# alpha-davidson/TensorBNN

Measured on AMD Instinct MI355X. Metric: leapfrog steps/sec (whole node), higher is better.
Workload: dtype f32

## Files before the change

### tensorbnn_amd/csrc/kernels_hmc.hpp

```cpp
#pragma once
#include "common.hpp"
#include "update_ops.hpp"

template <int UC = UPD_COLS, int UG = UPD_GROUPS>
__global__ __launch_bounds__(UC * UG) void k_update(
    NetDev nd, int mode, float eps, const float* __restrict__ eta,
    const float* __restrict__ slabs, int nslab, int pitch,
    const float* __restrict__ q_cur, const float* __restrict__ g_cur,
    float* __restrict__ q, float* __restrict__ p, float* __restrict__ g,
    const int* __restrict__ imgmap, float* __restrict__ qimg, float* __restrict__ gd = nullptr, int img_floats = 0,
    const StepCtl* __restrict__ ctl = nullptr, int t = 0)
{
    asm volatile("" :: "s"(mode), "s"(ctl), "s"(slabs), "s"(nslab), "s"(pitch), "s"(eta), "s"(q), "s"(p), "s"(imgmap), "s"(nd.P), "s"(nd.nl));
    if (ctl && mode != UPD_GRAD_ONLY) {
        const StepCtl me = ctl[blockIdx.y];
        eps = me.eps;
        if (t == 0) mode = UPD_FIRST;
        else if (t < me.L) mode = UPD_MID;
        else if (t == me.L) mode = UPD_LAST;
        else return;
    }
    if (blockIdx.y) {
        const size_t c = blockIdx.y, cp = c * (size_t)nd.P;
        eta += c * nd.H; slabs += c * (size_t)nslab * pitch;
// ... 31 lines not shown
        int w = y;
        for (; w + 12 < nslab; w += 16) {
            s0 += src[(size_t)w * pitch]; s1 += src[(size_t)(w + 4) * pitch];
            s2 += src[(size_t)(w + 8) * pitch]; s3 += src[(size_t)(w + 12) * pitch];
        }
        for (; w < nslab; w += 4) s0 += src[(size_t)w * pitch];
    }
    part[y][x] = (s0 + s1) + (s2 + s3);
    __syncthreads();
    if (y == 0 && j < P) {
        const float v = (part[0][x] + part[1][x]) + (part[2][x] + part[3][x]);
        if (out) out[j] = v;
        if (outd) outd[j] = (double)v;
    }
}

__global__ __launch_bounds__(256) void k_shard_pack(int P, const float* __restrict__ row, const double* __restrict__ pstat, int nstat,
                                                     double* __restrict__ buf, double sub) {
    __shared__ double red[4];
    const int j = blockIdx.x * blockDim.x + threadIdx.x;
    if (row && j < P) buf[j] = (double)row[j];
    if (blockIdx.x == 0) {
        double st = 0.0;
        for (int w = threadIdx.x; w < nstat; w += blockDim.x) st += pstat[w];
        st = block_sum(st, red);
        if (threadIdx.x == 0) buf[P] = st - sub;
    }
}
__global__ __launch_bounds__(256) void k_shard_unpack(int P, const double* __restrict__ buf, float* __restrict__ row,
                                                       double* __restrict__ stat_red) {
    const int j = blockIdx.x * blockDim.x + threadIdx.x;
    if (j < P) row[j] = (float)buf[j];
    if (j == 0) stat_red[0] = buf[P];
}

#define LIKC_BLOCKS 64
__global__ __launch_bounds__(256) void k_pois_const(const float* __restrict__ Y, const float* __restrict__ w, long n, int d_out,
                                                     double* __restrict__ out, double r) {
    __shared__ double red[4];
    double c = 0.0, bad = 0.0;
    const long nel = n * d_out;
    const double lgr = r > 0.0 ? lgamma(r) : 0.0;
    for (long el = (long)blockIdx.x * 256 + threadIdx.x; el < nel; el += (long)LIKC_BLOCKS * 256) {
        const float y = Y[el];
        if (!(y >= 0.f && y < INFINITY)) { bad += 1.0; continue; }
        const double wt = w ? (double)w[el / d_out] : 1.0;
        double t = lgamma((double)y + 1.0);
        if (r > 0.0) t += lgr - lgamma((double)y + r);
        c += wt * t;
    }
    c = block_sum(c, red);
    bad = block_sum(bad, red);
    if (threadIdx.x == 0) { out[2 * blockIdx.x] = c; out[2 * blockIdx.x + 1] = bad; }
}

__global__ __launch_bounds__(256) void k_copy_f32(int n, const float* __restrict__ src, float* __restrict__ dst) {
    const int j = blockIdx.x * blockDim.x + threadIdx.x;
    if (j < n) dst[j] = src[j];
}

__global__ __launch_bounds__(256) void k_make_image(int P, const float* __restrict__ q,
                                                    const int* __restrict__ imgmap, float* __restrict__ qimg,
                                                    long q_stride = 0, long img_stride = 0) {
    q += (size_t)blockIdx.y * q_stride; qimg += (size_t)blockIdx.y * img_stride;
    const int j = blockIdx.x * blockDim.x + threadIdx.x;
    if (j < P) { const float v = q[j]; qimg[imgmap[j]] = v; const int m1 = imgmap[P + j]; if (m1 >= 0) qimg[m1] = v; }
}

__device__ __forceinline__ double data_logp(const NetDev& nd, const float* __restrict__ eta, double stat, double n, double lik_c) {
    if (nd.lik == TBNN_LIK_POISSON) return stat - lik_c;
    if (nd.lik == TBNN_LIK_NEG_BINOMIAL) return stat - lik_c;
    if (nd.lik == TBNN_LIK_BERNOULLI || nd.lik == TBNN_LIK_CATEGORICAL) return stat;
    if (nd.lik == TBNN_LIK_HETERO_GAUSSIAN) return stat - 0.5 * 1.8378770664093453  * n;
    if (nd.lik == TBNN_LIK_STUDENT_T) {
        const double nu = (double)nd.lik_df, s = (double)lik_sigma(nd, eta);
        const double c = lgamma(0.5 * (nu + 1.0)) - lgamma(0.5 * nu) - 0.5 * log(nu * 3.14159265358979323846) - log(s);
        return n * (double)nd.d_out * c - 0.5 * (nu + 1.0) * stat;
    }
    const double s = (double)lik_sigma(nd, eta);
    const double nel = (double)n * (double)nd.d_out;
    return -0.5 * (2.0 * nel * log(s) + stat / (s * s) + nel * 1.8378770664093453 );
}

__device__ __forceinline__ double prior_logp_partial(const NetDev& nd, const float* __restrict__ eta,
                                                     const float* __restrict__ q) {
    double acc = 0.0;
    for (int l = 0; l < nd.nl; ++l) {
        for (int part = 0; part < 2; ++part) {
            const int off = part ? nd.offB[l] : nd.offW[l];
            const int cnt = part ? nd.out[l] : nd.out[l] * nd.in[l];
            const float loc = eta[4 * l + 2 * part];
            const float gg = eta[4 * l + 2 * part + 1];
            const float scale = gg * gg;
            if (nd.prior[l] == TBNN_PRIOR_CAUCHY) {
                const float lb = logf(3.14159265358979323846f * scale);
                for (int e = threadIdx.x; e < cnt; e += blockDim.x) {
                    const float z = (q[off + e] - loc) / scale;
                    acc += (double)(logf(1.f + z * z) - lb);
                }
            } else {
                const float s = fminf(fmaxf(scale, 1e-8f), 1e8f);
                for (int e = threadIdx.x; e < cnt; e += blockDim.x) {
                    const float d = (q[off + e] - loc) / s;
                    acc += -0.5 * (double)(d * d);
                }
                if (threadIdx.x == 0) acc += -0.5 * (2.0 * (double)logf(s) + 1.8378770664093453);
            }
        }
    }
    return acc;
}

__global__ __launch_bounds__(1024) void k_begin(
    NetDev nd, const float* __restrict__ p0_inj, const float* __restrict__ logu_inj,
    uint32_t epoch, uint32_t key0, uint32_t key1, float* __restrict__ p, Scal* __restrict__ sc, uint32_t seed_hi = 0)
{
    __shared__ double red[16];
    if (blockIdx.y) {
        const uint32_t c = blockIdx.y;
        key1 = (((key1 ^ seed_hi) + c) ^ seed_hi);
        p += (size_t)c * nd.P; sc += c;
        if (p0_inj) p0_inj += (size_t)c * nd.P;
        if (logu_inj) logu_inj += c;
    }
    double k = 0.0;
    if (p0_inj) {
        for (int j = threadIdx.x; j < nd.P; j += blockDim.x) { const float v = p0_inj[j]; p[j] = v; k += (double)v * (double)v; }
    } else {
        for (int b = threadIdx.x; 4 * b < nd.P; b += blockDim.x) {
            float v[4];
            philox_normal4((uint32_t)b, epoch, PURPOSE_MOMENTUM, key0, key1, v);
#pragma unroll
            for (int i = 0; i < 4; ++i)
                if (4 * b + i < nd.P) { p[4 * b + i] = v[i]; k += (double)v[i] * (double)v[i]; }
        }
    }
    k = block_sum(k, red);
    if (threadIdx.x == 0) {
        sc->k0 = 0.5 * k;
        sc->logu = logu_inj ? (double)logu_inj[0] : (double)philox_logu(epoch, PURPOSE_LOGU, key0, key1);
    }
}

enum { EN_CUR = 0, EN_NEW = 1, EN_TRACE = 2, EN_REFRESH = 3 };
__global__ __launch_bounds__(1024) void k_energy(
    NetDev nd, int which, const float* __restrict__ eta, const float* __restrict__ q,
    const float* __restrict__ p, const float* q_cur,
    const double* __restrict__ partial_stat, int nslab, double n, double lik_c,
    Scal* __restrict__ sc, double* __restrict__ trace_slot,
    Scal* __restrict__ commit_out = nullptr, const float* __restrict__ g = nullptr, float* q_cur_w = nullptr,
    float* __restrict__ g_cur = nullptr, const float* __restrict__ gd = nullptr, float* __restrict__ gd_cur = nullptr,
    const Scal* __restrict__ only_if_accepted = nullptr)
{
    __shared__ double red[16];
    __shared__ int s_acc;
    if (only_if_accepted && !only_if_accepted[blockIdx.y].accepted) return;
    if (blockIdx.y) {
        const size_t c = blockIdx.y, cp = c * (size_t)nd.P;
        eta += c * nd.H; q += cp; p += cp; q_cur += cp; partial_stat += c * PSTAT_CAP; sc += c;
        if (commit_out) commit_out += c;
        if (g) g += cp;
        if (q_cur_w) q_cur_w += cp;
        if (g_cur) g_cur += cp;
        if (gd) gd += cp;
        if (gd_cur) gd_cur += cp;
    }
    double st = 0.0;
    if (which != EN_REFRESH) {
        for (int w = threadIdx.x; w < nslab; w += blockDim.x) st += partial_stat[w];
        st = block_sum(st, red);
    }
    double pr = prior_logp_partial(nd, eta, q);
    pr = block_sum(pr, red);
    double k1 = 0.0, d2 = 0.0;
    if (which == EN_NEW) {
        for (int j = threadIdx.x; j < nd.P; j += blockDim.x) {
            const double pj = (double)p[j];
            const double dq = (double)q[j] - (double)q_cur[j];
            k1 += pj * pj;
            d2 += dq * dq;
        }
        k1 = block_sum(k1, red);
        d2 = block_sum(d2, red);
    }
    const bool commit = which == EN_NEW && commit_out != nullptr;
    if (threadIdx.x != 0 && !commit) return;
    if (threadIdx.x == 0) {
        if (which == EN_REFRESH) { st = sc->stat_cur; which = EN_CUR; }
        const double lp = pr + data_logp(nd, eta, st, n, lik_c);
        if (which == EN_TRACE) { *trace_slot = lp; return; }
        if (which == EN_CUR) {
            sc->stat_cur = st; sc->prior_cur = pr; sc->logp_cur = lp;
            if (trace_slot) *trace_slot = lp;
            return;
        }
        sc->stat_new = st; sc->prior_new = pr; sc->logp_new = lp;
        sc->k1 = 0.5 * k1; sc->d2 = d2;
        double lar = lp - sc->logp_cur + sc->k0 - 0.5 * k1;
        if (!isfinite(lar)) lar = -INFINITY;
        sc->lar = lar;
        const int acc = sc->logu < lar ? 1 : 0;
        sc->accepted = acc;
        sc->sjd = acc ? d2 : 0.0;
        if (trace_slot) *trace_slot = lp;
        if (commit) {
            *commit_out = *sc;
            if (acc) { sc->stat_cur = st; sc->prior_cur = pr; sc->logp_cur = lp; }
            s_acc = acc;
        }
    }
    if (!commit) return;
    __syncthreads();
    if (!s_acc) return;
    for (int j = threadIdx.x; j < nd.P; j += blockDim.x) { q_cur_w[j] = q[j]; g_cur[j] = g[j]; gd_cur[j] = gd[j]; }
}

__global__ __launch_bounds__(256) void k_commit(
    int P, const Scal* __restrict__ sc, const float* __restrict__ q, const float* __restrict__ g,
    float* __restrict__ q_cur, float* __restrict__ g_cur, const float* __restrict__ gd, float* __restrict__ gd_cur)
{
    const size_t c = blockIdx.y, cp = c * (size_t)P;
    if (!sc[c].accepted) return;
    const int j = blockIdx.x * blockDim.x + threadIdx.x;
    if (j < P) { q_cur[cp + j] = q[cp + j]; g_cur[cp + j] = g[cp + j]; gd_cur[cp + j] = gd[cp + j]; }
}

__global__ __launch_bounds__(256) void k_refresh_grad_after_hyper(
    NetDev nd, const float* __restrict__ eta, const float* __restrict__ q_cur,
    const float* __restrict__ gd_cur, float* __restrict__ g_cur, const Scal* __restrict__ hyper_rec = nullptr)
{
    if (blockIdx.y) {
        const size_t c = blockIdx.y, cp = c * (size_t)nd.P;
        eta += c * nd.H; q_cur += cp; gd_cur += cp; g_cur += cp;
    }
    if (hyper_rec && !hyper_rec[blockIdx.y].accepted) return;
    const int j = blockIdx.x * blockDim.x + threadIdx.x;
    if (j >= nd.P) return;
    const float sn = lik_sigma(nd, eta);
    const float inv_var = nd.lik == TBNN_LIK_GAUSSIAN ? 1.f / (sn * sn) : 1.f;
    int prior; float loc, scale;
    prior_params(nd, eta, j, prior, loc, scale);
    g_cur[j] = gd_cur[j] * inv_var + prior_grad(prior, loc, scale, q_cur[j]);
}
__global__ void k_commit_scal(Scal* __restrict__ sc, Scal* __restrict__ host_copy) {
    if (threadIdx.x != 0) return;
    sc += blockIdx.x; host_copy += blockIdx.x;
    *host_copy = *sc;
    if (sc->accepted) { sc->stat_cur = sc->stat_new; sc->prior_cur = sc->prior_new; sc->logp_cur = sc->logp_new; }
}

__global__ void k_trace_logp_cur(const Scal* __restrict__ sc, double* __restrict__ slot) {
    if (threadIdx.x == 0 && blockIdx.x == 0) *slot = sc->logp_cur;
}

__global__ void k_debug_draw(uint32_t epoch, uint32_t purpose, uint32_t key0, uint32_t key1, int n,
                             float* __restrict__ normals, float* __restrict__ logu) {
    const int j = blockIdx.x * blockDim.x + threadIdx.x;
    if (j < n) normals[j] = philox_normal((uint32_t)j, epoch, purpose, key0, key1);
    if (j == 0) logu[0] = philox_logu(epoch, purpose + 1u, key0, key1);
}
```

### tensorbnn_amd/csrc/tbnn_api.hip

```cpp
#include <hip/hip_runtime.h>
#include <rccl/rccl.h>
#include <dlfcn.h>
#include <cmath>
#include <cstdio>
#include <cstdlib>
#include <cstring>
#include <memory>
#include <new>
#include <string>
#include <utility>
#include <vector>

#include "common.hpp"
#include "kernels_generic.hpp"
#include "kernels_hmc.hpp"
#include "kernels_hyper.hpp"
#include "kernels_layered.hpp"
#include "kernels_ensemble.hpp"
#include "kernels_optim.hpp"
#include "aot_ops.hpp"
#include <mutex>

static thread_local std::string g_err;
static int fail(int code, const std::string& msg) { g_err = msg; return code; }
// ... 611 lines not shown
    HIPCHK(hipMemcpyAsync(h->tmp + h->nd.P, h->eta, (size_t)h->nd.H * sizeof(float), hipMemcpyDeviceToDevice, h->stream));
    NCCLCHK(g_rccl.AllGather(h->tmp, d_out, per, ncclFloat, c->comm, h->stream));
    if (host_out) HIPCHK(hipMemcpyAsync(host_out, d_out, tot * sizeof(float), hipMemcpyDeviceToHost, h->stream));
    HIPCHK(hipStreamSynchronize(h->stream));
    return 0;
}
extern "C" int tbnn_set_row_shard(tbnn_handle h, tbnn_comm_handle c, int64_t n_total) {
    NEED(h);
    ONE_CHAIN(h, "tbnn_set_row_shard");
    HIPCHK(hipSetDevice(h->device));
    HIPCHK(hipStreamSynchronize(h->stream));
    if (c && n_total < 1) return fail(-1, "n_total must be >= 1");
    if (c && h->dYw) return fail(-1, "tbnn_set_row_shard: the handle has row weights (tbnn_set_row_weights): weighted row sharding needs the weight sum of all ranks");
    h->shard = c; h->n_total = c ? (long)n_total : 0;
    h->cur_valid = false;
    return 0;
}
static inline double rows_total(const tbnn_ctx* h) { return h->dYw ? h->wsum : (double)(h->shard ? h->n_total : h->n); }
static inline double lik_const(const tbnn_ctx* h) { return h->shard ? 0.0 : h->lik_c; }
static inline const float* pass_Y(const tbnn_ctx* h) { return h->dYw ? h->dYw : h->dY; }
static inline const float* pass_w(const tbnn_ctx* h) { return h->dYw ? h->dYw + (size_t)h->n * h->nd.d_out : nullptr; }
static inline int stat_entries(const tbnn_ctx* h) { return h->shard ? 1 : h->grid; }
static inline const double* stat_ptr(const tbnn_ctx* h) { return h->shard ? h->pstat_red : h->pstat; }
static inline const float* grad_slabs(const tbnn_ctx* h) { return (h->shard && !h->be->slab_is_grad_row()) ? h->grow : h->slabs; }
static inline int grad_nslab(const tbnn_ctx* h) { return h->shard ? 1 : h->nslab; }

static hipEvent_t profile_begin(tbnn_ctx* h, int steps) {
    if (!(h->profile > 0 && (h->launch_no++ % h->profile) == 0)) return nullptr;
    if (h->pev_used + 2 > h->pev.size()) {
        hipEvent_t a = nullptr, b = nullptr;
        hipEventCreate(&a); hipEventCreate(&b); h->pev.emplace_back(a); h->pev.emplace_back(b);
    }
    const hipEvent_t a = h->pev[h->pev_used], b = h->pev[h->pev_used + 1];
    h->pev_used += 2;
    h->pev_div.push_back(steps);
    hipEventRecord(a, h->stream);
    return b;
}
static int launch_fwd_bwd(tbnn_ctx* h, const float* q, const float* eta, const StepCtl* ctl = nullptr, int t = 0) {
    const float* img = nullptr;
    const int C = h->C;
    const long imgS = h->img_floats, slabS = (long)h->nslab * h->pitch;
    if (h->imgmap) {
        if (q == h->q && h->q_img_valid) img = h->qimg;
        else {
            hipLaunchKernelGGL(k_make_image, dim3((h->nd.P + 255) / 256, C), dim3(256), 0, h->stream, h->nd.P, q, h->imgmap, h->qimg_cur, (long)h->nd.P, imgS);
            img = h->qimg_cur;
        }
    }
    const hipEvent_t prof_end = profile_begin(h, 1);
    const PassArgs pa = {img, imgS, q, eta, (long)h->nd.H, h->dX, pass_Y(h), pass_w(h), h->n, h->slabs, slabS, h->pitch, h->pstat, C, ctl, t, h->ctl_host};
    if (const int rc = h->be->fwd_bwd(h->stream, pa)) return rc;
    if (h->shard) {
        const bool dense = h->be->slab_is_grad_row();
        float* row = dense ? h->slabs : h->grow;
        const int P = h->nd.P;
        if (!dense)
            hipLaunchKernelGGL(k_slab_reduce, dim3((P + 63) / 64), dim3(64, 4), 0, h->stream, (const float*)h->slabs, h->nslab,
                               h->pitch, P, (float*)nullptr, h->shard_buf);
        hipLaunchKernelGGL(k_shard_pack, dim3((P + 255) / 256), dim3(256), 0, h->stream, P, dense ? (const float*)row : (const float*)nullptr,
                           (const double*)h->pstat, h->grid, h->shard_buf, h->lik_c);
        NCCLCHK(g_rccl.AllReduce(h->shard_buf, h->shard_buf, (size_t)P + 1, ncclDouble, ncclSum, h->shard->comm, h->stream));
        hipLaunchKernelGGL(k_shard_unpack, dim3((P + 255) / 256), dim3(256), 0, h->stream, P, (const double*)h->shard_buf, row, h->pstat_red);
    }
    if (prof_end) hipEventRecord(prof_end, h->stream);
    HIPCHK(hipGetLastError());
    return 0;
}
static void launch_update(tbnn_ctx* h, int mode, float eps, const float* eta, float* q, float* g, const StepCtl* ctl = nullptr, int t = 0) {
    const bool big = h->nd.P >= UPD_BIG_P;
    const int ucols = big ? UPD_COLS_BIG : UPD_COLS;
    const int gx = (h->pitch / 4 + ucols - 1) / ucols;
    const bool img = h->imgmap && q == h->q;
    float* gd = g == h->g_cur ? h->gd_cur : (g == h->g ? h->gd : nullptr);
    if (big)
        hipLaunchKernelGGL((k_update<UPD_COLS_BIG, UPD_GROUPS_BIG>), dim3(gx, h->C), dim3(UPD_COLS_BIG, UPD_GROUPS_BIG), 0, h->stream, h->nd, mode, eps, eta,
                           grad_slabs(h), grad_nslab(h), h->pitch, h->q_cur, h->g_cur, q, h->p, g, img ? h->imgmap : nullptr, h->qimg, gd, h->img_floats, ctl, t);
    else
        hipLaunchKernelGGL((k_update<UPD_COLS, UPD_GROUPS>), dim3(gx, h->C), dim3(UPD_COLS, UPD_GROUPS), 0, h->stream, h->nd, mode, eps, eta, grad_slabs(h),
                           grad_nslab(h), h->pitch, h->q_cur, h->g_cur, q, h->p, g, img ? h->imgmap : nullptr, h->qimg, gd, h->img_floats, ctl, t);
    if (img && (mode == UPD_FIRST || mode == UPD_MID)) h->q_img_valid = true;
}
static void launch_energy(tbnn_ctx* h, int which, const float* eta, const float* q, double* slot) {
    hipLaunchKernelGGL(k_energy, dim3(1, h->C), dim3(1024), 0, h->stream, h->nd, which, eta, q, h->p, h->q_cur, stat_ptr(h),
                       stat_entries(h), rows_total(h), lik_const(h), h->sc, slot);
}

static int ensure_current(tbnn_ctx* h, double* slot) {
    if (h->cur_valid) return 0;
    int rc = launch_fwd_bwd(h, h->q_cur, h->eta);
    if (rc) return rc;
    launch_update(h, UPD_GRAD_ONLY, 0.f, h->eta, h->q_cur, h->g_cur);
    launch_energy(h, EN_CUR, h->eta, h->q_cur, slot);
    h->cur_valid = true;
    return 0;
}
static float drain_profile(tbnn_ctx* h) {
    double tot = 0.0; int cnt = 0;
    for (size_t i = 0; i + 1 < h->pev_used; i += 2) {
        float ms = 0.f;
        const int div = i / 2 < h->pev_div.size() ? h->pev_div[i / 2] : 1;
        if (hipEventElapsedTime(&ms, h->pev[i], h->pev[i + 1]) == hipSuccess) { tot += ms * 1000.0 / (div > 0 ? div : 1); ++cnt; }
    }
    h->pev_used = 0;
    h->pev_div.clear();
    return cnt ? (float)(tot / cnt) : 0.f;
}

static int stage_theta(tbnn_ctx* h, const float* theta, const float** dq) {
    *dq = h->q_cur;
    if (!theta) return 0;
    HIPCHK(hipMemcpyAsync(h->q, theta, (size_t)h->nd.P * sizeof(float), hipMemcpyHostToDevice, h->stream));
    *dq = h->q; h->q_img_valid = false;
    return 0;
}

extern "C" int tbnn_logp_grad(tbnn_handle h, const float* theta, const float* eta, double* logp, float* grad,
                              double* stat) {
    NEED(h);
    ONE_CHAIN(h, "tbnn_logp_grad");
    if (!h->dX) return fail(-1, "tbnn_set_data has not been called");
    HIPCHK(hipSetDevice(h->device));
    const NetDev& nd = h->nd;
    const float* dq = nullptr;
    const float* de = h->eta;
    if (const int rc = stage_theta(h, theta, &dq)) return rc;
    if (eta) { HIPCHK(hipMemcpyAsync(h->tmp + nd.P, eta, (size_t)nd.H * sizeof(float), hipMemcpyHostToDevice, h->stream)); de = h->tmp + nd.P; }
    int rc = launch_fwd_bwd(h, dq, de);
    if (rc) return rc;
    const int gx = (h->pitch / 4 + UPD_COLS - 1) / UPD_COLS;
    hipLaunchKernelGGL((k_update<UPD_COLS, UPD_GROUPS>), dim3(gx), dim3(UPD_COLS, UPD_GROUPS), 0, h->stream, nd, (int)UPD_GRAD_ONLY, 0.f, de, grad_slabs(h), grad_nslab(h),
                       h->pitch, h->q_cur, h->g_cur, const_cast<float*>(dq), h->p, h->tmp, (const int*)nullptr, (float*)nullptr, (float*)nullptr);
    HIPCHK(h->trace.grow(2, 4096));
    hipLaunchKernelGGL(k_energy, dim3(1), dim3(1024), 0, h->stream, nd, (int)EN_TRACE, de, dq, h->p, h->q_cur, stat_ptr(h),
                       stat_entries(h), rows_total(h), lik_const(h), h->sc, h->trace);
    HIPCHK(hipGetLastError());
    double lp = 0.0;
    HIPCHK(hipMemcpyAsync(&lp, h->trace, sizeof(double), hipMemcpyDeviceToHost, h->stream));
    if (grad) HIPCHK(hipMemcpyAsync(grad, h->tmp, (size_t)nd.P * sizeof(float), hipMemcpyDeviceToHost, h->stream));
    std::vector<double> ps;
    if (stat) { ps.resize(stat_entries(h)); HIPCHK(hipMemcpyAsync(ps.data(), stat_ptr(h), ps.size() * sizeof(double), hipMemcpyDeviceToHost, h->stream)); }
    HIPCHK(hipStreamSynchronize(h->stream));
    if (h->profile) drain_profile(h);
    if (logp) *logp = lp;
    if (stat) {
        double s = 0; for (double v : ps) s += v;
        *stat = s - lik_const(h);
        if (nd.lik == TBNN_LIK_HETERO_GAUSSIAN) *stat -= 0.5 * 1.8378770664093453  * rows_total(h);
    }
    return 0;
}

extern "C" int tbnn_forward(tbnn_handle h, const float* theta, const float* X, int64_t n, float* out) {
    NEED(h);
    if (!theta) ONE_CHAIN(h, "tbnn_forward at the chain's own state");
    if (!X || !out || n < 1) return fail(-1, "forward: null pointer or n < 1");
    HIPCHK(hipSetDevice(h->device));
    const NetDev& nd = h->nd;
    const float* dq = nullptr;
    if (const int rc = stage_theta(h, theta, &dq)) return rc;
    Buf<float> dXf, dOut;
    HIPCHK(dXf.alloc((size_t)n * nd.d_in));
    HIPCHK(dOut.alloc((size_t)n * nd.d_out));
    HIPCHK(hipMemcpyAsync(dXf, X, (size_t)n * nd.d_in * sizeof(float), hipMemcpyHostToDevice, h->stream));
    if (const int rc = h->be->forward(h->stream, 1, dq, dXf, (long)n, dOut, h->imgmap, h->qimg_cur)) return rc;
    HIPCHK(hipMemcpyAsync(out, dOut, (size_t)n * nd.d_out * sizeof(float), hipMemcpyDeviceToHost, h->stream));
    HIPCHK(hipStreamSynchronize(h->stream));
    return 0;
}

extern "C" int tbnn_set_validation(tbnn_handle h, const float* X, const float* Y, int64_t n) {
    NEED(h);
    if (!X || !Y || n < 1) return fail(-1, "set_validation: null pointer or n < 1");
    HIPCHK(hipSetDevice(h->device));
    HIPCHK(hipStreamSynchronize(h->stream));
    h->dXv.reset(); h->dYv.reset();
    HIPCHK(h->dXv.alloc((size_t)n * h->nd.d_in));
    HIPCHK(h->dYv.alloc((size_t)n * h->nd.d_out));
    HIPCHK(hipMemcpy(h->dXv, X, (size_t)n * h->nd.d_in * sizeof(float), hipMemcpyHostToDevice));
    HIPCHK(hipMemcpy(h->dYv, Y, (size_t)n * h->nd.d_out * sizeof(float), hipMemcpyHostToDevice));
    h->nv = (long)n;
    return 0;
}

static int predict_resident(tbnn_ctx* h, int which, const float* theta, long* n_out) {
    const NetDev& nd = h->nd;
    if (!theta) ONE_CHAIN(h, "tbnn_predict / tbnn_metrics at the chain's own state");
    const float* dX = which ? h->dXv : h->dX;
    const long n = which ? h->nv : h->n;
    if (!dX || n < 1) return fail(-1, which ? "tbnn_set_validation has not been called" : "tbnn_set_data has not been called");
    const float* dq = nullptr;
    if (const int rc = stage_theta(h, theta, &dq)) return rc;
    const size_t need = (size_t)n * nd.d_out;
    HIPCHK(h->fbuf.grow(need, need));
    *n_out = n;
    return h->be->forward(h->stream, 1, dq, dX, n, h->fbuf, h->imgmap, h->qimg_cur);
}

extern "C" int tbnn_predict(tbnn_handle h, int which, const float* theta, float* out) {
    NEED(h);
    if (which != 0 && which != 1) return fail(-1, "which must be 0 (training rows) or 1 (validation rows)");
    HIPCHK(hipSetDevice(h->device));
    long n = 0;
    int rc = predict_resident(h, which, theta, &n);
    if (rc) return rc;
    if (out) HIPCHK(hipMemcpyAsync(out, h->fbuf, (size_t)n * h->nd.d_out * sizeof(float), hipMemcpyDeviceToHost, h->stream));
    HIPCHK(hipStreamSynchronize(h->stream));
    return 0;
}

#include "ensemble_api.hpp"

extern "C" int tbnn_metrics(tbnn_handle h, int which, const float* theta, float mean, float sd, int exp_pred, int exp_real,
                            double out3[3]) {
    NEED(h);
    if (!out3) return fail(-1, "null out3");
    if (which != 0 && which != 1) return fail(-1, "which must be 0 (training rows) or 1 (validation rows)");
    HIPCHK(hipSetDevice(h->device));
    long n = 0;
    int rc = predict_resident(h, which, theta, &n);
    if (rc) return rc;
    const int MB = 256;
    HIPCHK(h->mpart.grow(3 * MB, 3 * MB));
    const int d_cmp = h->nd.lik == TBNN_LIK_HETERO_GAUSSIAN ? 1 : h->nd.d_out;
    const long tot = n * d_cmp;
    const int grid = (int)std::min<long>(MB, (tot + 255) / 256);
    hipLaunchKernelGGL(k_metrics, dim3(grid), dim3(256), 0, h->stream, (const float*)h->fbuf, (const float*)(which ? h->dYv : h->dY), n,
                       d_cmp, h->nd.d_out, mean, sd, exp_pred, exp_real, h->mpart);
    HIPCHK(hipGetLastError());
    std::vector<double> part(3 * (size_t)grid);
    HIPCHK(hipMemcpyAsync(part.data(), h->mpart, part.size() * sizeof(double), hipMemcpyDeviceToHost, h->stream));
    HIPCHK(hipStreamSynchronize(h->stream));
    double a[3] = {0, 0, 0};
    for (int b = 0; b < grid; ++b) for (int k = 0; k < 3; ++k) a[k] += part[3 * b + k];
    for (int k = 0; k < 3; ++k) out3[k] = a[k] / (double)tot;
    return 0;
}

static int enqueue_transition(tbnn_ctx* h, float eps, int L, const float* d_p0, const float* d_logu, double* d_trace,
                              Scal* d_out, const StepCtl* ctl = nullptr) {
    const NetDev& nd = h->nd;
    const bool cached = h->cur_valid;
    int rc = ensure_current(h, d_trace);
    if (rc) return rc;
    if (d_trace && cached) hipLaunchKernelGGL(k_trace_logp_cur, dim3(1), dim3(64), 0, h->stream, (const Scal*)h->sc, d_trace);
    hipLaunchKernelGGL(k_begin, dim3(1, h->C), dim3(1024), 0, h->stream, nd, d_p0, d_logu, h->epoch, h->key0, h->key1, h->p, h->sc, h->seed_hi);
    launch_update(h, UPD_FIRST, eps, h->eta, h->q, h->g, ctl, 0);
    const bool traj = h->traj && !d_trace && L >= 1 && h->n <= h->be->traj_max_rows() && !h->shard;
    h->last_path = traj ? "trajectory" : "per-step";
    if (traj) {
        const hipEvent_t prof_end = profile_begin(h, L);
        const int trc = h->be->trajectory(h->stream, h->C, h->qimg, (long)h->img_floats, h->eta, h->dX, h->dY, h->n, h->q, h->p, h->g, h->gd, h->imgmap, h->pstat,
                                          stat_entries(h), eps, L, ctl);
        if (prof_end) hipEventRecord(prof_end, h->stream);
        if (trc)
            return fail(-2, "trajectory kernel launch failed");
        h->q_img_valid = false;
    }
    for (int t = 1; t <= L && !traj; ++t) {
        rc = launch_fwd_bwd(h, h->q, h->eta, ctl, t);
        if (rc) return rc;
        if (d_trace && t < L) {
            launch_update(h, UPD_GRAD_ONLY, 0.f, h->eta, h->q, h->g);
            launch_energy(h, EN_TRACE, h->eta, h->q, d_trace + t);
        }
        launch_update(h, t < L ? UPD_MID : UPD_LAST, eps, h->eta, h->q, h->g, ctl, t);
    }
    if (h->merge_ends && nd.P <= 32768) {
        hipLaunchKernelGGL(k_energy, dim3(1, h->C), dim3(1024), 0, h->stream, h->nd, (int)EN_NEW, (const float*)h->eta, (const float*)h->q, (const float*)h->p,
                           (const float*)h->q_cur, stat_ptr(h), stat_entries(h), rows_total(h), lik_const(h), h->sc, d_trace ? d_trace + L : (double*)nullptr,
                           d_out, (const float*)h->g, h->q_cur, h->g_cur, (const float*)h->gd, h->gd_cur);
    } else {
        launch_energy(h, EN_NEW, h->eta, h->q, d_trace ? d_trace + L : nullptr);
        hipLaunchKernelGGL(k_commit, dim3((nd.P + 255) / 256, h->C), dim3(256), 0, h->stream, nd.P, (const Scal*)h->sc, (const float*)h->q, (const float*)h->g,
                           h->q_cur, h->g_cur, (const float*)h->gd, h->gd_cur);
        hipLaunchKernelGGL(k_commit_scal, dim3(h->C), dim3(64), 0, h->stream, h->sc, d_out);
    }
    HIPCHK(hipGetLastError());
    h->epoch += 1;
    return 0;
}

static void fill_out(const Scal& s, int L, float dev_us, float fb_us, tbnn_step_out* o) {
    o->accepted = s.accepted; o->n_leapfrog = L;
    o->log_accept_ratio = (float)s.lar;
    o->accept_prob = s.lar < 0 ? (float)exp(s.lar) : 1.f;
    o->logp_old = s.logp_cur; o->logp_new = s.logp_new;
    o->kinetic_old = s.k0; o->kinetic_new = s.k1;
    o->sjd = s.sjd; o->device_us = dev_us; o->fwdbwd_us = fb_us;
}

extern "C" int tbnn_hmc_step(tbnn_handle h, float eps, int32_t L, const float* p0, const float* log_u,
                             tbnn_step_out* out, double* trace_logp) {
    NEED(h);
    if (!h->dX) return fail(-1, "tbnn_set_data has not been called");
    if (L < 1) return fail(-1, "L must be >= 1");
    if (h->C > 1 && (p0 || log_u || trace_logp)) return fail(-1, "hmc_step on a multi-chain handle: no injected draws, no trace (out: one record per chain)");
    HIPCHK(hipSetDevice(h->device));
    const NetDev& nd = h->nd;
    const float* d_p0 = nullptr; const float* d_lu = nullptr;
    if (p0) { HIPCHK(hipMemcpyAsync(h->p0_inj, p0, (size_t)nd.P * sizeof(float), hipMemcpyHostToDevice, h->stream)); d_p0 = h->p0_inj; }
    if (log_u) { HIPCHK(hipMemcpyAsync(h->logu_inj, log_u, sizeof(float), hipMemcpyHostToDevice, h->stream)); d_lu = h->logu_inj; }
    double* d_trace = nullptr;
    if (trace_logp) {
        HIPCHK(h->trace.grow((size_t)L + 1, (size_t)L + 1 + 4096));
        d_trace = h->trace;
    }
    HIPCHK(hipEventRecord(h->ev0, h->stream));
    int rc = enqueue_transition(h, eps, L, d_p0, d_lu, d_trace, h->sc_out);
    if (rc) return rc;
    HIPCHK(hipEventRecord(h->ev1, h->stream));
    HIPCHK(hipMemcpyAsync(h->sc_host, h->sc_out, (size_t)h->C * sizeof(Scal), hipMemcpyDeviceToHost, h->stream));
    if (trace_logp) HIPCHK(hipMemcpyAsync(trace_logp, h->trace, (size_t)(L + 1) * sizeof(double), hipMemcpyDeviceToHost, h->stream));
    HIPCHK(hipStreamSynchronize(h->stream));
    float ms = 0.f; hipEventElapsedTime(&ms, h->ev0, h->ev1);
    const float fb = h->profile ? drain_profile(h) : 0.f;
    if (out)
        for (int c = 0; c < h->C; ++c) fill_out(h->sc_host[c], L, ms * 1000.f, fb, out + c);
    return 0;
}

static int grow_records(tbnn_ctx* h, int n_epochs) {
    const size_t need = (size_t)n_epochs * h->C;
    HIPCHK(h->d_recs.grow(need, std::max<size_t>(need, 64)));
    HIPCHK(h->h_recs.grow(need, std::max<size_t>(need, 64)));
    return 0;
}
extern "C" int tbnn_hmc_run(tbnn_handle h, float eps, int32_t L, int32_t n_epochs, tbnn_step_out* outs) {
    NEED(h);
    if (!h->dX) return fail(-1, "tbnn_set_data has not been called");
    if (L < 1 || n_epochs < 1) return fail(-1, "L and n_epochs must be >= 1");
    if ((long long)n_epochs * (long long)h->C > (1LL << 24)) return fail(-1, "n_epochs x chains exceeds 2^24 records per call: split the run");
    HIPCHK(hipSetDevice(h->device));
    const int C = h->C;
    if (const int rc = grow_records(h, n_epochs)) return rc;
    HIPCHK(hipEventRecord(h->ev0, h->stream));
    for (int e = 0; e < n_epochs; ++e) {
        int rc = enqueue_transition(h, eps, L, nullptr, nullptr, nullptr, h->d_recs + (size_t)e * C);
        if (rc) return rc;
    }
    HIPCHK(hipEventRecord(h->ev1, h->stream));
    HIPCHK(hipMemcpyAsync(h->h_recs, h->d_recs, (size_t)n_epochs * C * sizeof(Scal), hipMemcpyDeviceToHost, h->stream));
    HIPCHK(hipStreamSynchronize(h->stream));
    float ms = 0.f; hipEventElapsedTime(&ms, h->ev0, h->ev1);
    const float fb = h->profile ? drain_profile(h) : 0.f;
    if (outs)
        for (int c = 0; c < C; ++c)
            for (int e = 0; e < n_epochs; ++e) fill_out(h->h_recs[(size_t)e * C + c], L, ms * 1000.f / n_epochs, fb, outs + (size_t)c * n_epochs + e);
    return 0;
}

static int stage_ctl(tbnn_ctx* h, const float* eps, const int32_t* L, int* Lmax) {
// ... 150 lines not shown
    const size_t B = (size_t)h->C * h->nd.P * sizeof(float);
    if (m) HIPCHK(hipMemcpyAsync(m, h->opt_m, B, hipMemcpyDeviceToHost, h->stream));
    if (v) HIPCHK(hipMemcpyAsync(v, h->opt_v, B, hipMemcpyDeviceToHost, h->stream));
    if (vhat) HIPCHK(hipMemcpyAsync(vhat, h->opt_vhat, B, hipMemcpyDeviceToHost, h->stream));
    if (g) HIPCHK(hipMemcpyAsync(g, h->opt_g, B, hipMemcpyDeviceToHost, h->stream));
    HIPCHK(hipStreamSynchronize(h->stream));
    if (t) *t = (int32_t)h->opt_t;
    return 0;
}

extern "C" int tbnn_hyper_logp_grad(tbnn_handle h, const float* eta, double* logp, float* grad) {
    NEED(h);
    ONE_CHAIN(h, "tbnn_hyper_logp_grad");
    if (!h->dX) return fail(-1, "tbnn_set_data has not been called");
    HIPCHK(hipSetDevice(h->device));
    const NetDev& nd = h->nd;
    int rc = ensure_current(h, nullptr);
    if (rc) return rc;
    float* de = h->eta;
    if (eta) { HIPCHK(hipMemcpyAsync(h->tmp + nd.P, eta, (size_t)nd.H * sizeof(float), hipMemcpyHostToDevice, h->stream)); de = h->tmp + nd.P; }
    hipLaunchKernelGGL(k_hyper, dim3(1), dim3(HYP_THREADS), 0, h->stream, nd, (int)HYP_EVAL, 0.f, 0, de, h->q_cur, rows_total(h),
                       (const float*)nullptr, (const float*)nullptr, 0u, h->key0, h->key1, h->sc, h->hyp_ws, h->sc_out);
    HIPCHK(hipGetLastError());
    std::vector<float> ws(hyper_ws_bytes(nd) / sizeof(float));
    HIPCHK(hipMemcpyAsync(ws.data(), h->hyp_ws, hyper_ws_bytes(nd), hipMemcpyDeviceToHost, h->stream));
    HIPCHK(hipMemcpyAsync(h->sc_host, h->sc_out, sizeof(Scal), hipMemcpyDeviceToHost, h->stream));
    HIPCHK(hipStreamSynchronize(h->stream));
    if (logp) *logp = h->sc_host[0].logp_new;
    if (grad) memcpy(grad, ws.data() + HYP_WS_GRAD * nd.H, (size_t)nd.H * sizeof(float));
    return 0;
}

static int hyper_step_impl(tbnn_handle h, float eps_h, const float* eps_each, int32_t L_h, const float* p0, const float* log_u, tbnn_step_out* out);
extern "C" int tbnn_hyper_step(tbnn_handle h, float eps_h, int32_t L_h, const float* p0, const float* log_u,
                               tbnn_step_out* out) {
    return hyper_step_impl(h, eps_h, nullptr, L_h, p0, log_u, out);
}
extern "C" int tbnn_hyper_step_each(tbnn_handle h, const float* eps_h, int32_t L_h, tbnn_step_out* out) {
    NEED(h);
    if (!eps_h) return fail(-1, "null eps_h array");
    return hyper_step_impl(h, 0.f, eps_h, L_h, nullptr, nullptr, out);
}
static int hyper_step_impl(tbnn_handle h, float eps_h, const float* eps_each, int32_t L_h, const float* p0, const float* log_u, tbnn_step_out* out) {
    NEED(h);
    if (!h->dX) return fail(-1, "tbnn_set_data has not been called");
    if (L_h < 1) return fail(-1, "L_h must be >= 1");
    if (h->C > 1 && (p0 || log_u)) return fail(-1, "hyper_step on a multi-chain handle: no injected draws (out: one record per chain)");
    HIPCHK(hipSetDevice(h->device));
    const NetDev& nd = h->nd;
    const int C = h->C;
    int rc = ensure_current(h, nullptr);
    if (rc) return rc;
    const float* d_p0 = nullptr; const float* d_lu = nullptr;
    if (p0) { HIPCHK(hipMemcpyAsync(h->p0_inj, p0, (size_t)nd.H * sizeof(float), hipMemcpyHostToDevice, h->stream)); d_p0 = h->p0_inj; }
    if (log_u) { HIPCHK(hipMemcpyAsync(h->logu_inj, log_u, sizeof(float), hipMemcpyHostToDevice, h->stream)); d_lu = h->logu_inj; }
    HIPCHK(hipMemcpyAsync(h->eta_prev, h->eta, (size_t)C * nd.H * sizeof(float), hipMemcpyDeviceToDevice, h->stream));
    const float* d_each = nullptr;
    if (eps_each) {
        memcpy(h->epsh_host, eps_each, (size_t)C * sizeof(float));
        HIPCHK(hipMemcpyAsync(h->epsh, h->epsh_host, (size_t)C * sizeof(float), hipMemcpyHostToDevice, h->stream));
        d_each = h->epsh;
    }
    HIPCHK(hipEventRecord(h->ev0, h->stream));
    const uint32_t ep = h->epoch > 0 ? h->epoch - 1 : 0;
    static_assert(sizeof(float) * 4 == 16, "hyper work space: 4 H floats per chain (hyper_ws_bytes)");
    hipLaunchKernelGGL(k_hyper, dim3(C), dim3(HYP_THREADS), 0, h->stream, nd, (int)HYP_STEP, eps_h, (int)L_h, h->eta, (const float*)h->q_cur, rows_total(h),
                       d_p0, d_lu, ep, h->key0, h->key1, h->sc, h->hyp_ws, h->sc_out, h->seed_hi, d_each);
    HIPCHK(hipGetLastError());
    HIPCHK(hipEventRecord(h->ev1, h->stream));
    HIPCHK(hipMemcpyAsync(h->sc_host, h->sc_out, (size_t)C * sizeof(Scal), hipMemcpyDeviceToHost, h->stream));
    HIPCHK(hipStreamSynchronize(h->stream));
    float ms = 0.f; hipEventElapsedTime(&ms, h->ev0, h->ev1);
    if (out)
        for (int c = 0; c < C; ++c) fill_out(h->sc_host[c], L_h, ms * 1000.f, 0.f, out + c);
    bool any = false;
    for (int c = 0; c < C; ++c) any = any || h->sc_host[c].accepted;
    if (any) {
        static const bool full = getenv("TBNN_HYPER_FULL_REFRESH") && atoi(getenv("TBNN_HYPER_FULL_REFRESH"));
        if (full || !h->cur_valid) h->cur_valid = false;
        else {
            const Scal* gate = C > 1 ? (const Scal*)h->sc_out : (const Scal*)nullptr;
            hipLaunchKernelGGL(k_refresh_grad_after_hyper, dim3((nd.P + 255) / 256, C), dim3(256), 0, h->stream, nd,
                               (const float*)h->eta, (const float*)h->q_cur, (const float*)h->gd_cur, h->g_cur, gate);
            hipLaunchKernelGGL(k_energy, dim3(1, C), dim3(1024), 0, h->stream, nd, (int)EN_REFRESH, (const float*)h->eta,
                               (const float*)h->q_cur, (const float*)h->p, (const float*)h->q_cur,
                               stat_ptr(h), stat_entries(h), rows_total(h), lik_const(h), h->sc, (double*)nullptr,
                               (Scal*)nullptr, (const float*)nullptr, (float*)nullptr, (float*)nullptr, (const float*)nullptr, (float*)nullptr, gate);
            HIPCHK(hipGetLastError());
        }
    }
    return 0;
}

extern "C" int tbnn_hyper_probs_many(tbnn_handle h, const int32_t* priors, const float* thetas, int64_t theta_stride,
                                     const float* etas, int64_t eta_stride, int32_t m, double* out) {
    NEED(h);
    const NetDev& nd0 = h->nd;
    if (!thetas || !etas || !out || m < 1 || theta_stride < nd0.P || eta_stride < 4 * nd0.nl)
        return fail(-1, "hyper_probs_many: null pointer, m < 1, theta_stride < P or eta_stride < 4 * layers");
    NetDev nd = nd0;
    if (priors)
        for (int l = 0; l < nd.nl; ++l) {
            if (priors[l] != TBNN_PRIOR_CAUCHY && priors[l] != TBNN_PRIOR_GAUSSIAN) return fail(-1, "hyper_probs_many: unknown prior");
            nd.prior[l] = priors[l];
        }
    HIPCHK(hipSetDevice(h->device));
    Buf<float> dTh, dEt; Buf<double> dOut;
    const int chunk = (int)std::min<size_t>((size_t)m, std::max<size_t>(1, ((size_t)1 << 28) / (size_t)nd.P));
    HIPCHK(dTh.alloc((size_t)chunk * nd.P));
    HIPCHK(dEt.alloc((size_t)chunk * 4 * nd.nl));
    HIPCHK(dOut.alloc((size_t)chunk));
    for (int i0 = 0; i0 < m; i0 += chunk) {
        const int c = std::min(chunk, m - i0);
        HIPCHK(hipMemcpy2DAsync(dTh, (size_t)nd.P * sizeof(float), thetas + (size_t)i0 * theta_stride, (size_t)theta_stride * sizeof(float),
                                (size_t)nd.P * sizeof(float), (size_t)c, hipMemcpyHostToDevice, h->stream));
        HIPCHK(hipMemcpy2DAsync(dEt, (size_t)4 * nd.nl * sizeof(float), etas + (size_t)i0 * eta_stride, (size_t)eta_stride * sizeof(float),
                                (size_t)4 * nd.nl * sizeof(float), (size_t)c, hipMemcpyHostToDevice, h->stream));
        hipLaunchKernelGGL(k_hyper_probs, dim3(c), dim3(256), 0, h->stream, nd, (const float*)dTh, (long)nd.P, (const float*)dEt, (long)(4 * nd.nl), dOut);
        HIPCHK(hipGetLastError());
        HIPCHK(hipMemcpyAsync(out + i0, dOut, (size_t)c * sizeof(double), hipMemcpyDeviceToHost, h->stream));
        HIPCHK(hipStreamSynchronize(h->stream));
    }
    return 0;
}

extern "C" int tbnn_export_sample_device(tbnn_handle h, float* d_out) {
    NEED(h); if (!d_out) return fail(-1, "null d_out");
    ONE_CHAIN(h, "tbnn_export_sample_device");
    HIPCHK(hipSetDevice(h->device));
    HIPCHK(hipMemcpyAsync(d_out, h->q_cur, (size_t)h->nd.P * sizeof(float), hipMemcpyDeviceToDevice, h->stream));
    HIPCHK(hipMemcpyAsync(d_out + h->nd.P, h->eta, (size_t)h->nd.H * sizeof(float), hipMemcpyDeviceToDevice, h->stream));
    HIPCHK(hipStreamSynchronize(h->stream));
    return 0;
}

extern "C" int tbnn_debug_momentum(tbnn_handle h, float* p_out) {
    NEED(h); if (!p_out) return fail(-1, "null p_out");
    ONE_CHAIN(h, "tbnn_debug_momentum");
    HIPCHK(hipSetDevice(h->device));
    HIPCHK(hipMemcpyAsync(p_out, h->p, (size_t)h->nd.P * sizeof(float), hipMemcpyDeviceToHost, h->stream));
    HIPCHK(hipStreamSynchronize(h->stream));
    return 0;
}

extern "C" int tbnn_debug_draw(tbnn_handle h, uint32_t epoch, uint32_t purpose, int32_t n, float* out_normals,
                               float* out_log_u) {
    NEED(h);
    if (n < 1 || !out_normals) return fail(-1, "debug_draw: bad arguments");
    HIPCHK(hipSetDevice(h->device));
    Buf<float> d;
    HIPCHK(d.alloc((size_t)n + 1));
    hipLaunchKernelGGL(k_debug_draw, dim3((n + 255) / 256), dim3(256), 0, h->stream, epoch, purpose, h->key0, h->key1, (int)n, d, d + n);
    HIPCHK(hipGetLastError());
    std::vector<float> host(n + 1);
    HIPCHK(hipMemcpyAsync(host.data(), d, (size_t)(n + 1) * sizeof(float), hipMemcpyDeviceToHost, h->stream));
    HIPCHK(hipStreamSynchronize(h->stream));
    memcpy(out_normals, host.data(), (size_t)n * sizeof(float));
    if (out_log_u) *out_log_u = host[n];
    return 0;
}

extern "C" int tbnn_debug_stamps(tbnn_handle h, uint64_t* out5) {
    if (!out5) return fail(-1, "null out16");
    NEED(h);
    const FusedOps* ops = h->be->ops();
    if (!ops || ops != narrow_find(h->nd) || !h->dX || h->C > 1) return fail(-1, "debug_stamps: narrow fast kernel + data required");
    HIPCHK(hipSetDevice(h->device));
// ... 55 lines not shown
```

Baseline: 22220.

## Preload energy-kernel operands into registers and shared memory, fuse block reductions

Restructures k_energy so each thread issues all of its global loads (q, p, q_cur, g, gd, eta, partial stats, Scal) up front into register arrays, stages q and eta in shared memory for the prior pass, and merges the separate block reductions into one multi-value reduction. The commit copy reuses the register-held values instead of reloading them. k_begin gets the same early-load treatment. The goal is to cut the serialized global-load latency and the repeated __syncthreads reductions in a single-block-per-chain kernel, at the cost of more registers and about 24KB of shared memory per block.

```diff
diff --git a/tensorbnn_amd/csrc/kernels_hmc.hpp b/tensorbnn_amd/csrc/kernels_hmc.hpp
--- a/tensorbnn_amd/csrc/kernels_hmc.hpp
+++ b/tensorbnn_amd/csrc/kernels_hmc.hpp
@@ -137,8 +137,8 @@
     return -0.5 * (2.0 * nel * log(s) + stat / (s * s) + nel * 1.8378770664093453 );
 }
 
-__device__ __forceinline__ double prior_logp_partial(const NetDev& nd, const float* __restrict__ eta,
-                                                     const float* __restrict__ q) {
+template <class QAt>
+__device__ __forceinline__ double prior_logp_partial_of(const NetDev& nd, const float* __restrict__ eta, QAt qat, int stride) {
     double acc = 0.0;
     for (int l = 0; l < nd.nl; ++l) {
         for (int part = 0; part < 2; ++part) {
@@ -149,14 +149,14 @@
             const float scale = gg * gg;
             if (nd.prior[l] == TBNN_PRIOR_CAUCHY) {
                 const float lb = logf(3.14159265358979323846f * scale);
-                for (int e = threadIdx.x; e < cnt; e += blockDim.x) {
-                    const float z = (q[off + e] - loc) / scale;
+                for (int e = threadIdx.x; e < cnt; e += stride) {
+                    const float z = (qat(off + e) - loc) / scale;
                     acc += (double)(logf(1.f + z * z) - lb);
                 }
             } else {
                 const float s = fminf(fmaxf(scale, 1e-8f), 1e8f);
-                for (int e = threadIdx.x; e < cnt; e += blockDim.x) {
-                    const float d = (q[off + e] - loc) / s;
+                for (int e = threadIdx.x; e < cnt; e += stride) {
+                    const float d = (qat(off + e) - loc) / s;
                     acc += -0.5 * (double)(d * d);
                 }
                 if (threadIdx.x == 0) acc += -0.5 * (2.0 * (double)logf(s) + 1.8378770664093453);
@@ -165,12 +165,41 @@
     }
     return acc;
 }
+__device__ __forceinline__ double prior_logp_partial(const NetDev& nd, const float* __restrict__ eta,
+                                                     const float* __restrict__ q) {
+    return prior_logp_partial_of(nd, eta, [q](int i) { return q[i]; }, (int)blockDim.x);
+}
+
+#define EN_THREADS 1024
+#define EN_CAP 6
+static_assert(EN_CAP == 6, "EN_PIN names the elements");
+#define EN_PIN(a) asm volatile("" : "+v"(a[0]), "+v"(a[1]), "+v"(a[2]), "+v"(a[3]), "+v"(a[4]), "+v"(a[5]))
+
+template <int N, int NW = EN_THREADS / 64>
+__device__ __forceinline__ void block_sum_n(double (&v)[N], double (*red)[16]) {
+    const int lane = threadIdx.x & 63, w = threadIdx.x >> 6, nw = NW;
+#pragma unroll
+    for (int i = 0; i < N; ++i) v[i] = wave_sum(v[i]);
+    if (lane == 0) {
+#pragma unroll
+        for (int i = 0; i < N; ++i) red[i][w] = v[i];
+    }
+    __syncthreads();
+#pragma unroll
+    for (int i = 0; i < N; ++i) v[i] = 0.0;
+    if (w == 0) {
+#pragma unroll
+        for (int i = 0; i < N; ++i) v[i] = lane < nw ? red[i][lane] : 0.0;
+#pragma unroll
+        for (int i = 0; i < N; ++i) v[i] = wave_sum(v[i]);
+    }
+}
 
 __global__ __launch_bounds__(1024) void k_begin(
     NetDev nd, const float* __restrict__ p0_inj, const float* __restrict__ logu_inj,
     uint32_t epoch, uint32_t key0, uint32_t key1, float* __restrict__ p, Scal* __restrict__ sc, uint32_t seed_hi = 0)
 {
-    __shared__ double red[16];
+    __shared__ double red[1][16];
     if (blockIdx.y) {
         const uint32_t c = blockIdx.y;
         key1 = (((key1 ^ seed_hi) + c) ^ seed_hi);
@@ -178,11 +207,19 @@
         if (p0_inj) p0_inj += (size_t)c * nd.P;
         if (logu_inj) logu_inj += c;
     }
+    double logu = 0.0;
+    if (threadIdx.x == 0) logu = logu_inj ? (double)logu_inj[0] : (double)philox_logu(epoch, PURPOSE_LOGU, key0, key1);
     double k = 0.0;
     if (p0_inj) {
-        for (int j = threadIdx.x; j < nd.P; j += blockDim.x) { const float v = p0_inj[j]; p[j] = v; k += (double)v * (double)v; }
+        float v[EN_CAP];
+#pragma unroll
+        for (int i = 0; i < EN_CAP; ++i) { const int j = threadIdx.x + i * EN_THREADS; v[i] = j < nd.P ? p0_inj[j] : 0.f; }
+        EN_PIN(v);
+#pragma unroll
+        for (int i = 0; i < EN_CAP; ++i) { const int j = threadIdx.x + i * EN_THREADS; if (j < nd.P) { p[j] = v[i]; k += (double)v[i] * (double)v[i]; } }
+        for (int j = threadIdx.x + EN_CAP * EN_THREADS; j < nd.P; j += EN_THREADS) { const float x = p0_inj[j]; p[j] = x; k += (double)x * (double)x; }
     } else {
-        for (int b = threadIdx.x; 4 * b < nd.P; b += blockDim.x) {
+        for (int b = threadIdx.x; 4 * b < nd.P; b += EN_THREADS) {
             float v[4];
             philox_normal4((uint32_t)b, epoch, PURPOSE_MOMENTUM, key0, key1, v);
 #pragma unroll
@@ -190,10 +227,11 @@
                 if (4 * b + i < nd.P) { p[4 * b + i] = v[i]; k += (double)v[i] * (double)v[i]; }
         }
     }
-    k = block_sum(k, red);
+    double kv[1] = {k};
+    block_sum_n<1>(kv, red);
     if (threadIdx.x == 0) {
-        sc->k0 = 0.5 * k;
-        sc->logu = logu_inj ? (double)logu_inj[0] : (double)philox_logu(epoch, PURPOSE_LOGU, key0, key1);
+        sc->k0 = 0.5 * kv[0];
+        sc->logu = logu;
     }
 }
 
@@ -207,8 +245,12 @@
     float* __restrict__ g_cur = nullptr, const float* __restrict__ gd = nullptr, float* __restrict__ gd_cur = nullptr,
     const Scal* __restrict__ only_if_accepted = nullptr)
 {
-    __shared__ double red[16];
+    __shared__ double red[4][16];
     __shared__ int s_acc;
+    __shared__ float s_q[EN_CAP * EN_THREADS];
+    __shared__ float s_eta[4 * TBNN_MAX_LAYERS + 4];
+    asm volatile("" :: "s"(which), "s"(eta), "s"(q), "s"(p), "s"(q_cur), "s"(partial_stat), "s"(nslab), "s"(sc), "s"(commit_out), "s"(g), "s"(gd),
+                 "s"(only_if_accepted), "s"(nd.P), "s"(nd.H), "s"(nd.nl), "s"(nd.offW[0]), "s"(nd.offB[0]), "s"(nd.out[0]), "s"(nd.in[0]), "s"(nd.prior[0]));
     if (only_if_accepted && !only_if_accepted[blockIdx.y].accepted) return;
     if (blockIdx.y) {
         const size_t c = blockIdx.y, cp = c * (size_t)nd.P;
@@ -220,46 +262,107 @@
         if (gd) gd += cp;
         if (gd_cur) gd_cur += cp;
     }
+    const int tid = threadIdx.x;
+    const bool is_new = which == EN_NEW;
+    const bool commit = is_new && commit_out != nullptr;
+    const bool has_st = which != EN_REFRESH && tid < nslab;
+    double st0 = 0.0;
+    if (has_st) st0 = partial_stat[tid];
+    float qv[EN_CAP], pv[EN_CAP], qc[EN_CAP], gv[EN_CAP], gdv[EN_CAP];
+#pragma unroll
+    for (int i = 0; i < EN_CAP; ++i) {
+        const int j = tid + i * EN_THREADS;
+        qv[i] = pv[i] = qc[i] = gv[i] = gdv[i] = 0.f;
+        if (j < nd.P) qv[i] = q[j];
+    }
+    if (is_new) {
+#pragma unroll
+        for (int i = 0; i < EN_CAP; ++i) {
+            const int j = tid + i * EN_THREADS;
+            if (j < nd.P) { pv[i] = p[j]; qc[i] = q_cur[j]; }
+        }
+    }
+    if (commit) {
+#pragma unroll
+        for (int i = 0; i < EN_CAP; ++i) {
+            const int j = tid + i * EN_THREADS;
+            if (j < nd.P) { gv[i] = g[j]; gdv[i] = gd[j]; }
+        }
+    }
+    float eta_v = 0.f;
+    if (tid < nd.H) eta_v = eta[tid];
+    Scal s0 = {};
+    if (tid == 0) s0 = *sc;
+    EN_PIN(qv); EN_PIN(pv); EN_PIN(qc); EN_PIN(gv); EN_PIN(gdv);
+    asm volatile("" : "+v"(eta_v), "+v"(st0));
+#pragma unroll
+    for (int i = 0; i < EN_CAP; ++i) {
+        const int j = tid + i * EN_THREADS;
+        if (j < nd.P) s_q[j] = qv[i];
+    }
+    if (tid < nd.H) s_eta[tid] = eta_v;
     double st = 0.0;
     if (which != EN_REFRESH) {
-        for (int w = threadIdx.x; w < nslab; w += blockDim.x) st += partial_stat[w];
-        st = block_sum(st, red);
-    }
-    double pr = prior_logp_partial(nd, eta, q);
-    pr = block_sum(pr, red);
+        if (has_st) st += st0;
+        for (int w = tid + EN_THREADS; w < nslab; w += EN_THREADS) st += partial_stat[w];
+    }
     double k1 = 0.0, d2 = 0.0;
-    if (which == EN_NEW) {
-        for (int j = threadIdx.x; j < nd.P; j += blockDim.x) {
+    if (is_new) {
+#pragma unroll
+        for (int i = 0; i < EN_CAP; ++i) {
+            const int j = tid + i * EN_THREADS;
+            if (j < nd.P) {
+                const double pj = (double)pv[i];
+                const double dq = (double)qv[i] - (double)qc[i];
+                k1 += pj * pj;
+                d2 += dq * dq;
+            }
+        }
+        for (int j = tid + EN_CAP * EN_THREADS; j < nd.P; j += EN_THREADS) {
             const double pj = (double)p[j];
             const double dq = (double)q[j] - (double)q_cur[j];
             k1 += pj * pj;
             d2 += dq * dq;
         }
-        k1 = block_sum(k1, red);
-        d2 = block_sum(d2, red);
-    }
-    const bool commit = which == EN_NEW && commit_out != nullptr;
-    if (threadIdx.x != 0 && !commit) return;
-    if (threadIdx.x == 0) {
-        if (which == EN_REFRESH) { st = sc->stat_cur; which = EN_CUR; }
-        const double lp = pr + data_logp(nd, eta, st, n, lik_c);
+    }
+    __syncthreads();
+    const float* sq = s_q;
+    double pr = prior_logp_partial_of(nd, s_eta, [sq, q](int i) { return i < EN_CAP * EN_THREADS ? sq[i] : q[i]; }, EN_THREADS);
+    if (is_new) {
+        double v[4] = {st, pr, k1, d2};
+        block_sum_n<4>(v, red);
+        st = v[0]; pr = v[1]; k1 = v[2]; d2 = v[3];
+    } else {
+        double v[2] = {st, pr};
+        block_sum_n<2>(v, red);
+        st = v[0]; pr = v[1];
+    }
+    if (tid != 0 && !commit) return;
+    if (tid == 0) {
+        if (which == EN_REFRESH) { st = s0.stat_cur; which = EN_CUR; }
+        const double lp = pr + data_logp(nd, s_eta, st, n, lik_c);
         if (which == EN_TRACE) { *trace_slot = lp; return; }
         if (which == EN_CUR) {
             sc->stat_cur = st; sc->prior_cur = pr; sc->logp_cur = lp;
             if (trace_slot) *trace_slot = lp;
             return;
         }
+        double lar = lp - s0.logp_cur + s0.k0 - 0.5 * k1;
+        if (!isfinite(lar)) lar = -INFINITY;
+        const int acc = s0.logu < lar ? 1 : 0;
+        s0.stat_new = st; s0.prior_new = pr; s0.logp_new = lp;
+        s0.k1 = 0.5 * k1; s0.d2 = d2;
+        s0.lar = lar;
+        s0.accepted = acc;
+        s0.sjd = acc ? d2 : 0.0;
         sc->stat_new = st; sc->prior_new = pr; sc->logp_new = lp;
-        sc->k1 = 0.5 * k1; sc->d2 = d2;
-        double lar = lp - sc->logp_cur + sc->k0 - 0.5 * k1;
-        if (!isfinite(lar)) lar = -INFINITY;
+        sc->k1 = s0.k1; sc->d2 = d2;
         sc->lar = lar;
-        const int acc = sc->logu < lar ? 1 : 0;
         sc->accepted = acc;
-        sc->sjd = acc ? d2 : 0.0;
+        sc->sjd = s0.sjd;
         if (trace_slot) *trace_slot = lp;
         if (commit) {
-            *commit_out = *sc;
+            *commit_out = s0;
             if (acc) { sc->stat_cur = st; sc->prior_cur = pr; sc->logp_cur = lp; }
             s_acc = acc;
         }
@@ -267,7 +370,12 @@
     if (!commit) return;
     __syncthreads();
     if (!s_acc) return;
-    for (int j = threadIdx.x; j < nd.P; j += blockDim.x) { q_cur_w[j] = q[j]; g_cur[j] = g[j]; gd_cur[j] = gd[j]; }
+#pragma unroll
+    for (int i = 0; i < EN_CAP; ++i) {
+        const int j = tid + i * EN_THREADS;
+        if (j < nd.P) { q_cur_w[j] = qv[i]; g_cur[j] = gv[i]; gd_cur[j] = gdv[i]; }
+    }
+    for (int j = tid + EN_CAP * EN_THREADS; j < nd.P; j += EN_THREADS) { q_cur_w[j] = q[j]; g_cur[j] = g[j]; gd_cur[j] = gd[j]; }
 }
 
 __global__ __launch_bounds__(256) void k_commit(
diff --git a/tensorbnn_amd/csrc/tbnn_api.hip b/tensorbnn_amd/csrc/tbnn_api.hip
--- a/tensorbnn_amd/csrc/tbnn_api.hip
+++ b/tensorbnn_amd/csrc/tbnn_api.hip
@@ -717,7 +717,7 @@
     if (img && (mode == UPD_FIRST || mode == UPD_MID)) h->q_img_valid = true;
 }
 static void launch_energy(tbnn_ctx* h, int which, const float* eta, const float* q, double* slot) {
-    hipLaunchKernelGGL(k_energy, dim3(1, h->C), dim3(1024), 0, h->stream, h->nd, which, eta, q, h->p, h->q_cur, stat_ptr(h),
+    hipLaunchKernelGGL(k_energy, dim3(1, h->C), dim3(EN_THREADS), 0, h->stream, h->nd, which, eta, q, h->p, h->q_cur, stat_ptr(h),
                        stat_entries(h), rows_total(h), lik_const(h), h->sc, slot);
 }
 
@@ -767,7 +767,7 @@
     hipLaunchKernelGGL((k_update<UPD_COLS, UPD_GROUPS>), dim3(gx), dim3(UPD_COLS, UPD_GROUPS), 0, h->stream, nd, (int)UPD_GRAD_ONLY, 0.f, de, grad_slabs(h), grad_nslab(h),
                        h->pitch, h->q_cur, h->g_cur, const_cast<float*>(dq), h->p, h->tmp, (const int*)nullptr, (float*)nullptr, (float*)nullptr);
     HIPCHK(h->trace.grow(2, 4096));
-    hipLaunchKernelGGL(k_energy, dim3(1), dim3(1024), 0, h->stream, nd, (int)EN_TRACE, de, dq, h->p, h->q_cur, stat_ptr(h),
+    hipLaunchKernelGGL(k_energy, dim3(1), dim3(EN_THREADS), 0, h->stream, nd, (int)EN_TRACE, de, dq, h->p, h->q_cur, stat_ptr(h),
                        stat_entries(h), rows_total(h), lik_const(h), h->sc, h->trace);
     HIPCHK(hipGetLastError());
     double lp = 0.0;
@@ -879,7 +879,7 @@
     int rc = ensure_current(h, d_trace);
     if (rc) return rc;
     if (d_trace && cached) hipLaunchKernelGGL(k_trace_logp_cur, dim3(1), dim3(64), 0, h->stream, (const Scal*)h->sc, d_trace);
-    hipLaunchKernelGGL(k_begin, dim3(1, h->C), dim3(1024), 0, h->stream, nd, d_p0, d_logu, h->epoch, h->key0, h->key1, h->p, h->sc, h->seed_hi);
+    hipLaunchKernelGGL(k_begin, dim3(1, h->C), dim3(EN_THREADS), 0, h->stream, nd, d_p0, d_logu, h->epoch, h->key0, h->key1, h->p, h->sc, h->seed_hi);
     launch_update(h, UPD_FIRST, eps, h->eta, h->q, h->g, ctl, 0);
     const bool traj = h->traj && !d_trace && L >= 1 && h->n <= h->be->traj_max_rows() && !h->shard;
     h->last_path = traj ? "trajectory" : "per-step";
@@ -902,7 +902,7 @@
         launch_update(h, t < L ? UPD_MID : UPD_LAST, eps, h->eta, h->q, h->g, ctl, t);
     }
     if (h->merge_ends && nd.P <= 32768) {
-        hipLaunchKernelGGL(k_energy, dim3(1, h->C), dim3(1024), 0, h->stream, h->nd, (int)EN_NEW, (const float*)h->eta, (const float*)h->q, (const float*)h->p,
+        hipLaunchKernelGGL(k_energy, dim3(1, h->C), dim3(EN_THREADS), 0, h->stream, h->nd, (int)EN_NEW, (const float*)h->eta, (const float*)h->q, (const float*)h->p,
                            (const float*)h->q_cur, stat_ptr(h), stat_entries(h), rows_total(h), lik_const(h), h->sc, d_trace ? d_trace + L : (double*)nullptr,
                            d_out, (const float*)h->g, h->q_cur, h->g_cur, (const float*)h->gd, h->gd_cur);
     } else {
@@ -1219,7 +1219,7 @@
             const Scal* gate = C > 1 ? (const Scal*)h->sc_out : (const Scal*)nullptr;
             hipLaunchKernelGGL(k_refresh_grad_after_hyper, dim3((nd.P + 255) / 256, C), dim3(256), 0, h->stream, nd,
                                (const float*)h->eta, (const float*)h->q_cur, (const float*)h->gd_cur, h->g_cur, gate);
-            hipLaunchKernelGGL(k_energy, dim3(1, C), dim3(1024), 0, h->stream, nd, (int)EN_REFRESH, (const float*)h->eta,
+            hipLaunchKernelGGL(k_energy, dim3(1, C), dim3(EN_THREADS), 0, h->stream, nd, (int)EN_REFRESH, (const float*)h->eta,
                                (const float*)h->q_cur, (const float*)h->p, (const float*)h->q_cur,
                                stat_ptr(h), stat_entries(h), rows_total(h), lik_const(h), h->sc, (double*)nullptr,
                                (Scal*)nullptr, (const float*)nullptr, (float*)nullptr, (float*)nullptr, (const float*)nullptr, (float*)nullptr, gate);
```

Result: no change. 22280, median of 6 (+0.3%).
